# SunYangtian/Splatter_A_Video

Hardware: AMD Instinct MI355X
Metric: rendered frames/sec fwd+bwd @480p, 300k Gaussians (higher is better)
Workload: dtype f32

## Files before the change

### splatter_a_video_amd/csrc/blend.hip

```cpp
#include <stdlib.h>

#include <utility>

#include "common.h"

__device__ __forceinline__ float exp2_guard(float pw, bool &ok) {
    ok = true;
    return __builtin_amdgcn_fmed3f(__builtin_amdgcn_exp2f(pw), 0.f, 1.f);
}

struct BlendArgs {
    int P, C;
    int c0, cn;
    const float2 *uv;
    const float *conic;
    const float *opacity;
    const float *feature;
    const float *bias;
    const int *idx_sorted;
    const int2 *tile_range;
    float bg;
    const float *bgc;
    int W, H, gx;
    int K, trunc;
// ... 352 lines not shown
__device__ __forceinline__ void keep_from_flags(TileLDS<CH, SB, COEF, XR, SWZ, RQL> &L, int tid, int nb, unsigned flags, Pred pred) {
    if (tid < SB) {
        unsigned kw = 0u;
        if (tid < nb) {
#pragma unroll
            for (int ww = 0; ww < 4; ++ww)
                if (((flags >> (8 * ww)) & 0xffu) && pred(tid, ww)) kw |= 1u << (8 * ww);
        }
        L.keep[tid] = kw;
    }
}

template <int SB, bool POS = true>
struct CarryLDS {
    static constexpr int CQ = 15;
    unsigned int pos4[POS ? SB : 1];
    int cslot[4][16];
    int more[4];
};

template <int CH, int SB, bool COEF, int XR, bool SWZ, int RQL, bool POS>
__device__ __forceinline__ int build_list_at(TileLDS<CH, SB, COEF, XR, SWZ, RQL> &L, CarryLDS<SB, POS> &C, int w, int lane, int base) {
    int cnt = 0;
#pragma unroll
    for (int r = 0; r < SB / WAVE; ++r) {
        const int e = r * WAVE + lane;
        const bool keep = ((L.keep[e] >> (8 * w)) & 0xffu) != 0u;
        const unsigned long long m = __ballot(keep);
        const int before = __builtin_amdgcn_mbcnt_hi((unsigned)(m >> 32), __builtin_amdgcn_mbcnt_lo((unsigned)m, 0u));
        if (keep) L.list[w][base + cnt + before] = (unsigned short)e;
        if (POS) reinterpret_cast<unsigned char *>(C.pos4)[4 * e + w] = keep ? (unsigned char)(base + cnt + before) : (unsigned char)255;
        cnt += __popcll(m);
    }
    if (lane < 16) L.list[w][base + cnt + lane] = (unsigned short)SB;
    __builtin_amdgcn_fence(__ATOMIC_RELEASE, "wavefront");
    __builtin_amdgcn_wave_barrier();
    return cnt;
}

template <int CH, int SB, bool COEF, int XR, bool SWZ, bool POS>
__device__ __forceinline__ void carry_out(TileLDS<CH, SB, COEF, XR, SWZ> &L, CarryLDS<SB, POS> &C, int w, int lane, int first, int left,
                                          int j0, int top, const int *slots) {
    constexpr int RQC = 2 + (CH + 3) / 4, CQ = CarryLDS<SB>::CQ;
    for (int idx = lane; idx < left * RQC; idx += WAVE) {
        const int k = idx / RQC, part = idx - k * RQC;
        const int e = L.list[w][first + k];
        float4 v = L.rec[L.part(e, part)];
        if (part == 1) v.w = __int_as_float(top - e);
        L.rec[L.part(SB + 1 + CQ * w + j0 + k, part)] = v;
    }
    int e = 0;
    if (lane < left) {
        e = L.list[w][first + lane];
        C.cslot[w][j0 + lane] = slots[top - e];
        if (POS) reinterpret_cast<unsigned char *>(C.pos4)[4 * e + w] = (unsigned char)255;
    }
    __builtin_amdgcn_fence(__ATOMIC_RELEASE, "wavefront");
    __builtin_amdgcn_wave_barrier();
    if (lane < left) L.list[w][j0 + lane] = (unsigned short)(SB + 1 + CQ * w + j0 + lane);
}

typedef float f32x4 __attribute__((ext_vector_type(4)));

template <int CH>
struct FwdCfg {
    static constexpr int SB = 128;
    static constexpr int U = 2;
    static constexpr int MINW = CH <= 4 ? 6 : CH <= 16 ? 4 : 3;
};

template <int CH, bool ENH, bool BIAS, bool EXACT>
__global__ void __launch_bounds__(256, FwdCfg<CH>::MINW)
blend_fwd_kernel(const BlendArgs B) {
    constexpr int SB = FwdCfg<CH>::SB;
    constexpr bool MF = CH >= 16 && !BIAS;
    constexpr int NCB = (CH + 15) / 16;
    constexpr int U = MF ? 4 : FwdCfg<CH>::U;
    constexpr int RB = Rec<CH>::RS * 4;
    constexpr int RM = RB / 32;
    constexpr int CS = (!BIAS && CH <= 4) ? 3 : 2;
    constexpr int CSB = 16 * CS;
    static_assert((SB + 1) * CSB <= 65536 && SB % U == 0 && RB % 32 == 0, "offsets must fit the 16-bit list entries");
    static_assert(BIAS ? CSB == 32 : true, "with a bias the list entries address the records (32-byte unit)");
    __shared__ TileLDS<CH, SB, !BIAS, 0, false, Rec<CH>::RQ, CS> L;
    __shared__ __attribute__((aligned(16))) unsigned int s_qlist[4][4][SB];
    __shared__ int s_done[4];
    const int tid = threadIdx.x, lane = tid & 63, w = tid >> 6;
    const int gtile = xcd_tile(blockIdx.x, gridDim.x);
    const int frame = gtile / B.T, tile = gtile - frame * B.T;
    const BlendArgs A = frame_args(B, frame);
    const int tx = tile % A.gx, ty = tile / A.gx;
    const int bx = tx * TILE + (w & 1) * 8, by = ty * TILE + (w >> 1) * 8;
    const int lx = MF ? ((lane >> 4) & 1) * 4 + (lane & 3) : (lane & 7);
    const int ly = MF ? (lane >> 5) * 4 + ((lane >> 2) & 3) : (lane >> 3);
    const int px = bx + lx, py = by + ly;
    const float pxf = (float)px, pyf = (float)py;
    const float x = (float)((w & 1) * 8 + lx) - 7.5f, y = (float)((w >> 1) * 8 + ly) - 7.5f;
    const float xx = x * x, xy = x * y, yy = y * y;
    const int cn = EXACT ? CH : A.cn;
    f32x4 D[MF ? 4 : 1][MF ? NCB : 1];
    if (MF) {
#pragma unroll
        for (int g = 0; g < 4; ++g)
#pragma unroll
            for (int c = 0; c < NCB; ++c) D[g][c] = f32x4{0.f, 0.f, 0.f, 0.f};
    }

    const bool inside = (px < A.W) && (py < A.H);
    float T = inside ? 1.0f : -1.0f, F[CH];
    int last = 0, layer = 0;
#pragma unroll
    for (int k = 0; k < CH; ++k) F[k] = 0.f;
    const int2 range = A.tile_range[tile];
    const int n = range.y - range.x;

    if (tid < Rec<CH>::RQ) L.rec[SB * Rec<CH>::RQ + tid] = make_float4(0.f, 0.f, 0.f, 0.f);
    if (!BIAS && tid < CS) L.coef[CS * SB + tid] = make_float4(tid == 0 ? -__builtin_inff() : 0.f, 0.f, 0.f, 0.f);
    auto pos = [n](int e, int b) { const int q = b * SB + e; return q < n ? q : -1; };
    Stager<CH, SB> st;
    st.load_ids(A, tid, range.x, pos, 0);
    st.load_payload(A, tid);
    st.load_ids(A, tid, range.x, pos, 1);

    for (int base = 0, batch = 0; base < n; base += SB, ++batch) {
        unsigned qd;
        {
            const unsigned long long dm = __ballot(T < 0.f);
            if (MF) {
                qd = ((dm & 0xffffull) == 0xffffull ? 1u : 0u) | (((dm >> 16) & 0xffffull) == 0xffffull ? 2u : 0u) |
                     (((dm >> 32) & 0xffffull) == 0xffffull ? 4u : 0u) | ((dm >> 48) == 0xffffull ? 8u : 0u);
            } else {
                constexpr unsigned long long Q0 = 0x000000000F0F0F0Full, Q1 = 0x00000000F0F0F0F0ull;
                qd = ((dm & Q0) == Q0 ? 1u : 0u) | ((dm & Q1) == Q1 ? 2u : 0u) | ((dm & (Q0 << 32)) == (Q0 << 32) ? 4u : 0u) |
                     ((dm & (Q1 << 32)) == (Q1 << 32) ? 8u : 0u);
            }
        }
        const bool alld = qd == 15u;
        if (lane == 0) s_done[w] = (int)qd;
        const int nb = imin_(SB, n - base);
        st.park(L, tid);
        st.load_payload(A, tid);
        st.load_ids(A, tid, range.x, pos, batch + 2);
        __syncthreads();
        if ((s_done[0] & s_done[1] & s_done[2] & s_done[3]) == 15) break;
        tile_cull<CH, SB, BIAS, true, !BIAS>(L, tid, nb, (float)(tx * TILE), (float)(ty * TILE), [&](int, int ww) -> unsigned { return 15u & ~(unsigned)s_done[ww]; },
                                             A.cull_flags ? A.cull_flags + range.x + base : nullptr);
        __syncthreads();
        if (!alld) {
            int cq[4];
#pragma unroll
            for (int q = 0; q < 4; ++q) cq[q] = 0;
#pragma unroll
            for (int r = 0; r < SB / WAVE; ++r) {
                const int e = r * WAVE + lane;
                const unsigned bits = (L.keep[e] >> (8 * w)) & 0xffu;
#pragma unroll
                for (int q = 0; q < 4; ++q) {
                    const bool keep = (bits >> q) & 1u;
                    const unsigned long long m = __ballot(keep);
                    const int before = __builtin_amdgcn_mbcnt_hi((unsigned)(m >> 32), __builtin_amdgcn_mbcnt_lo((unsigned)m, 0u));
                    if (keep) s_qlist[w][q][cq[q] + before] = (unsigned)(e * CSB);
                    cq[q] += __popcll(m);
                }
            }
            const int cnt = imax_(imax_(cq[0], cq[1]), imax_(cq[2], cq[3]));
            const int cntU = (cnt + U - 1) / U * U;
#pragma unroll
            for (int q = 0; q < 4; ++q)
#pragma unroll 1
                for (int i = cq[q] + lane; i < cntU; i += WAVE) s_qlist[w][q][i] = (unsigned)(SB * CSB);
            __builtin_amdgcn_fence(__ATOMIC_RELEASE, "wavefront");
            __builtin_amdgcn_wave_barrier();
            const int myq = MF ? (lane >> 4) : ((lane >> 2) & 1) + 2 * ((lane >> 5) & 1);
            const unsigned int *mylist = s_qlist[w][myq];
            const char *recb = reinterpret_cast<const char *>(L.rec);
            const char *cfb = reinterpret_cast<const char *>(L.coef);
            int lastoff = -1;
            const int chan_off = 4 * (lane & 15);
            const int chan_off1 = (16 + (lane & 15) < CH) ? 64 : -chan_off;
            for (int j0 = 0; j0 < cntU; j0 += U) {
                unsigned off[U];
                static_assert(U == 2 || U == 4, "a trip reads its list entries as one 8- or 16-byte word");
#pragma unroll
                for (int u = 0; u < U; ++u) off[u] = mylist[j0 + u];
                float bq[MF ? 4 : 1][MF ? NCB : 1];
                if constexpr (MF) {
#pragma unroll
                    for (int g = 0; g < 4; ++g) {
                        const unsigned og = s_qlist[w][g][j0 + (lane >> 4)];
                        const char *fb = recb + og * RM + 32 + chan_off;
#pragma unroll
                        for (int c = 0; c < NCB; ++c) bq[g][c] = *reinterpret_cast<const float *>(fb + (c == 0 ? 0 : chan_off1));
                    }
                }
                float4 g0[U], g1[U];
                float alpha[U];
                bool aok[U];
#pragma unroll
                for (int u = 0; u < U; ++u) {
                    const char *src = BIAS ? recb + off[u] * RM : cfb + off[u];
                    g0[u] = *reinterpret_cast<const float4 *>(src);
                    g1[u] = *reinterpret_cast<const float4 *>(src + 16);
                }
#pragma unroll
                for (int u = 0; u < U; ++u) {
                    if (BIAS) {
                        const float q = neg_power_factored(g0[u].x - pxf, g0[u].y - pyf, g0[u].z, g0[u].w, g1[u].x);
                        const float a = fminf(0.99f, __builtin_fmaf(g1[u].y, exp_neg(q), g1[u].z));
                        aok[u] = !(q < 0.f) && !(a < (1.0f / 255.0f));
                        alpha[u] = aok[u] ? a : 0.f;
                    } else {
                        const float pw = power_poly(g0[u], g1[u], x, y, xx, xy, yy);
                        bool pw_ok;
                        const float a = fminf(0.99f, exp2_guard(pw, pw_ok));
                        aok[u] = pw_ok && !(a < (1.0f / 255.0f));
                        alpha[u] = aok[u] ? a : 0.f;
                    }
                }
                float wq[MF ? U : 1];
#pragma unroll
                for (int u = 0; u < U; ++u) {
                    float f[MF ? 1 : CH];
                    if (!MF) {
                        if (CS == 3) asm volatile("" : "+v"(off[u]) : "v"(alpha[u]));
                        const float4 *fq = CS == 3 ? reinterpret_cast<const float4 *>(cfb + off[u] + 32)
                                                   : reinterpret_cast<const float4 *>(recb + off[u] * RM + 32);
#pragma unroll
                        for (int k = 0; k < CH; k += 4) {
                            const float4 v = fq[k / 4];
                            if (k + 0 < CH) f[k + 0] = v.x;
                            if (k + 1 < CH) f[k + 1] = v.y;
                            if (k + 2 < CH) f[k + 2] = v.z;
                            if (k + 3 < CH) f[k + 3] = v.w;
                        }
                    }
                    const float nT = T * (1.f - alpha[u]);
                    const bool sat = nT < 0.0001f;
                    const float wgt = sat ? 0.f : alpha[u] * T;
                    const bool app = CH <= 8 ? (aok[u] && !sat) : wgt > 0.f;
                    if (MF) {
                        wq[u] = wgt;
                    } else {
#pragma unroll
                        for (int k = 0; k < CH; ++k) F[k] += f[k] * wgt;
                    }
                    T = sat ? -fabsf(T) : nT;
                    lastoff = app ? (int)off[u] : lastoff;
                    if (ENH) {
                        if (app && (A.trunc || layer < A.K)) {
                            const size_t pix = (size_t)A.W * (size_t)py + px;
                            A.gs_idx[pix * A.K + layer] = __float_as_int(g1[u].w);
                            layer++;
                            if (A.trunc && layer >= A.K) T = -T;
                        }
                    }
                }
                if constexpr (MF) {
                    typedef unsigned u32x2_f __attribute__((ext_vector_type(2)));
                    const u32x2_f s02 = __builtin_amdgcn_permlane32_swap(__float_as_uint(wq[0]), __float_as_uint(wq[2]), false, false);
                    const u32x2_f s13 = __builtin_amdgcn_permlane32_swap(__float_as_uint(wq[1]), __float_as_uint(wq[3]), false, false);
                    const u32x2_f a01 = __builtin_amdgcn_permlane16_swap(s02[0], s13[0], false, false);
                    const u32x2_f a23 = __builtin_amdgcn_permlane16_swap(s02[1], s13[1], false, false);
                    const float Aq[4] = {__uint_as_float(a01[0]), __uint_as_float(a01[1]), __uint_as_float(a23[0]), __uint_as_float(a23[1])};
#pragma unroll
                    for (int g = 0; g < 4; ++g)
#pragma unroll
                        for (int c = 0; c < NCB; ++c) D[g][c] = __builtin_amdgcn_mfma_f32_16x16x4f32(Aq[g], bq[g][c], D[g][c], 0, 0, 0);
                }
            }
            last = lastoff >= 0 ? base + lastoff / CSB + 1 : last;
        }
        __syncthreads();
    }
    if constexpr (MF) {
        constexpr int ST = 36;
        static_assert(4 * 16 * ST * 4 <= (int)sizeof(L.rec), "four waves' quarter buffers fit the staged records");
        float *so = reinterpret_cast<float *>(L.rec) + w * (16 * ST);
#pragma unroll
        for (int g = 0; g < 4; ++g) {
#pragma unroll
            for (int c = 0; c < NCB; ++c)
#pragma unroll
                for (int j = 0; j < 4; ++j) so[(4 * (lane >> 4) + j) * ST + 16 * c + (lane & 15)] = D[g][c][j];
            __builtin_amdgcn_fence(__ATOMIC_RELEASE, "wavefront");
            __builtin_amdgcn_wave_barrier();
            const float4 *src = reinterpret_cast<const float4 *>(so + (lane & 15) * ST);
            const bool mine = (lane >> 4) == g;
#pragma unroll
            for (int k = 0; k < CH; k += 4) {
                const float4 v = src[k / 4];
                if (k + 0 < CH) F[k + 0] = mine ? v.x : F[k + 0];
                if (k + 1 < CH) F[k + 1] = mine ? v.y : F[k + 1];
                if (k + 2 < CH) F[k + 2] = mine ? v.z : F[k + 2];
                if (k + 3 < CH) F[k + 3] = mine ? v.w : F[k + 3];
            }
            __builtin_amdgcn_fence(__ATOMIC_RELEASE, "wavefront");
            __builtin_amdgcn_wave_barrier();
        }
    }
    if (inside) {
        const size_t HW = (size_t)A.H * A.W;
        const size_t pix = (size_t)A.W * (size_t)py + px;
        T = fabsf(T);
        A.final_T[pix] = T;
        A.ncontrib[pix] = last;
#pragma unroll
        for (int k = 0; k < CH; ++k)
            if (k < cn) A.out[(size_t)(A.c0 + k) * HW + pix] = F[k] + T * (A.bgc ? A.bgc[A.c0 + k] : A.bg);
        if (ENH)
            for (int l = layer; l < A.K; ++l) A.gs_idx[pix * A.K + l] = -1;
    }
}

#define DPP4(op)                                   \
    "v_add_f32_dpp %0, %0, %0 " op "\n\t"          \
    "v_add_f32_dpp %1, %1, %1 " op "\n\t"          \
    "v_add_f32_dpp %2, %2, %2 " op "\n\t"          \
    "v_add_f32_dpp %3, %3, %3 " op "\n\t"

__device__ __forceinline__ void wave_sum4_to_lane63(float &a, float &b, float &c, float &d) {
    asm volatile("s_nop 1\n\t" DPP4("row_shr:1 row_mask:0xf bank_mask:0xf bound_ctrl:1")
                     DPP4("row_shr:2 row_mask:0xf bank_mask:0xf bound_ctrl:1")
                         DPP4("row_shr:4 row_mask:0xf bank_mask:0xf bound_ctrl:1")
                             DPP4("row_shr:8 row_mask:0xf bank_mask:0xf bound_ctrl:1")
                                 DPP4("row_bcast:15 row_mask:0xa bank_mask:0xf")
                                     DPP4("row_bcast:31 row_mask:0xc bank_mask:0xf")
                 : "+v"(a), "+v"(b), "+v"(c), "+v"(d));
}

#define DPP3(op)                                   \
    "v_add_f32_dpp %0, %0, %0 " op "\n\t"          \
    "v_add_f32_dpp %1, %1, %1 " op "\n\t"          \
    "v_add_f32_dpp %2, %2, %2 " op "\n\t"

__device__ __forceinline__ void wave_sum3_to_lane63(float &a, float &b, float &c) {
    asm volatile("s_nop 1\n\t" DPP3("row_shr:1 row_mask:0xf bank_mask:0xf bound_ctrl:1")
                     DPP3("row_shr:2 row_mask:0xf bank_mask:0xf bound_ctrl:1")
                         DPP3("row_shr:4 row_mask:0xf bank_mask:0xf bound_ctrl:1")
                             DPP3("row_shr:8 row_mask:0xf bank_mask:0xf bound_ctrl:1")
                                 DPP3("row_bcast:15 row_mask:0xa bank_mask:0xf")
                                     DPP3("row_bcast:31 row_mask:0xc bank_mask:0xf")
                 : "+v"(a), "+v"(b), "+v"(c));
}

template <int N>
__device__ __forceinline__ void wave_sum_n_to_lane63(float (&v)[N]) {
    constexpr int B3 = (N >= 6 || N == 3) ? ((4 - (N & 3)) & 3) : 0;
    constexpr int N3 = 3 * B3;
    constexpr int N4 = (N - N3) & ~3;
#pragma unroll
    for (int k = 0; k < N4; k += 4) wave_sum4_to_lane63(v[k], v[k + 1], v[k + 2], v[k + 3]);
#pragma unroll
    for (int k = N4; k < N4 + N3; k += 3) wave_sum3_to_lane63(v[k], v[k + 1], v[k + 2]);
// ... 674 lines not shown
                        for (int i = 0; i < 4; ++i) {
                            const int c = 16 * q + 4 * kk + i;
                            if (c < CH) put(rec + NG + c, d_f[q][i]);
                        }
                }
            }
        }
        if (CARRY && p0 == 0) {
            __builtin_amdgcn_fence(__ATOMIC_RELEASE, "wavefront");
            __builtin_amdgcn_wave_barrier();
            if (nproc > 0)
                for (int idx = lane; idx < ncin * NC; idx += 64) {
                    const int k = idx / NC, c = idx - k * NC;
                    float *src = SHARED ? slab + (SB + CQ * w + k) * NCS + c : slab + idx;
                    __hip_atomic_fetch_add(pair_buf + (size_t)CL.cslot[w][k] * RST + c, *src, __ATOMIC_RELAXED,
                                           __HIP_MEMORY_SCOPE_AGENT);
                    if (SHARED) *src = 0.f;
                }
            const int left = total - nproc;
            if (left > 0) carry_out<CH, SB>(L, CL, w, lane, nproc > 0 ? nproc : ncin, nproc > 0 ? left : left - ncin,
                                            nproc > 0 ? 0 : ncin, top, slots);
            ncarry = left;
        }
        if (CARRY && !SHARED && lane == 0) CL.more[w] = nproc > p0 + CAP;
        if (p0 == 0) {
            load_slots();
            st.load_payload(A, tid);
            st.load_ids(A, tid, range.x, pos, batch + 2);
        }
        __syncthreads();
        if (ce < EPI) {
            const int lo = top - nb + 1;
            if (SHARED) {
#pragma unroll
                for (int r = 0; r < NPASS; ++r) {
                    const int ql = ce + r * EPI;
                    if (ql < nb) {
                        float *row = s_acc[0] + (nb - 1 - ql) * NCS + CW * cc;
                        const float v0 = row[0], v1 = row[CW > 1 ? 1 : 0], v2 = row[CW > 1 ? 2 : 0];
                        row[0] = 0.f;
                        if (CW > 1) { row[1] = 0.f; row[2] = 0.f; }
                        store_part(NPASS <= 3 ? sl[NPASS <= 3 ? r : 0] : slots[lo + ql], v0, v1, v2);
                    }
                }
            } else {
#pragma unroll
                for (int r = 0; r < NPASS; ++r) {
                    const int ql = ce + r * EPI;
                    if (ql < nb) {
                        const unsigned int p4 = CL.pos4[nb - 1 - ql];
                        float v[3] = {0.f, 0.f, 0.f};
#pragma unroll
                        for (int ww = 0; ww < 4; ++ww) {
                            const unsigned int pp = umin_(((p4 >> (8 * ww)) & 0xffu) - (unsigned)p0, (unsigned)CAP);
                            const float *row = s_acc[ww] + pp * NC + CW * cc;
#pragma unroll
                            for (int j = 0; j < 3; ++j)
                                if (CW * (TPR - 1) + j < NC || CW * cc + j < NC) v[j] += row[j];
                        }
                        const int slot = NPASS <= 3 ? sl[NPASS <= 3 ? r : 0] : slots[lo + ql];
                        if (p0 > 0) {
                            const float *old = pair_buf + (size_t)slot * RST + CW * cc;
#pragma unroll
                            for (int j = 0; j < 3; ++j)
                                if (CW * cc + j < NCP) v[j] += old[j];
                        }
                        store_part(slot, v[0], v[1], v[2]);
                    }
                }
            }
        }
        if (SHARED) break;
        const bool more = CARRY && (CL.more[0] | CL.more[1] | CL.more[2] | CL.more[3]);
        __syncthreads();
        if (!more) break;
        }
    }
    if (A.dbg_T_front) {
        const int px = bx + (lane & 7), py = by + (lane >> 3);
        if (px < A.W && py < A.H) A.dbg_T_front[(size_t)A.W * py + px] = s_pix[w][pixoff(lane) + PS + 2];
    }
}

template <int CH, bool ABS = false>
struct QuarterCfg {
    static_assert(CH <= 3 && Rec<CH>::RQ == 4 && Rec<CH>::CULL >= 11, "floats 11-15 of the record (cull parameters) are free for the coefficients");
    static constexpr int SB = 128;
    static constexpr int CAP = 80;
    static constexpr int MINW = 4;
    static constexpr int NG = GradLayout<ABS, false>::NG, NC = NG + CH, NCP = PAIR_STRIDE(NC);
    static constexpr int RW = ABS ? 16 : 12;
    static constexpr int PW = 8;
};

template <int CH, bool ABS, bool EXACT>
__global__ void __launch_bounds__(256, (QuarterCfg<CH, ABS>::MINW))
blend_bwd_quarter_kernel(const BlendArgs B) {
    using Cfg = QuarterCfg<CH, ABS>;
    constexpr int SB = Cfg::SB, CAP = Cfg::CAP, NCP = Cfg::NCP, RW = Cfg::RW, PW = Cfg::PW, RQ = 4;
    static_assert(SB <= 128 && CAP < 255, "list entries are (entry | position << 8) in 16 bits");
    __shared__ float4 s_rec[(SB + 1) * RQ];
    auto qpart = [](int e, int p) { return 4 * e + (p ^ ((e >> 2) & 3)); };
    __shared__ unsigned int s_keep[SB];
    __shared__ unsigned short s_qlist[4][4][CAP + 16];
    __shared__ unsigned int s_pos4[SB];
    __shared__ __attribute__((aligned(16))) float s_acc[4][(CAP + 1) * RW];
    constexpr int KS = 4 * PW + 8, GS = 4 * KS;
    __shared__ __attribute__((aligned(16))) float s_pix[4][4 * GS];
    auto pixoff = [](int q) { return (q >> 4) * GS + ((q >> 2) & 3) * KS + (q & 3) * PW; };
    __shared__ float s_mom[16 * 32];
    __shared__ int s_wmax[4];
    __shared__ int s_more[4];
    const int tid = threadIdx.x, lane = tid & 63, w = tid >> 6;
    const int gtile = xcd_tile(blockIdx.x, gridDim.x);
    const int frame = gtile / B.T, tile = gtile - frame * B.T;
    const BlendArgs A = frame_args(B, frame);
    const int RST = B.rec_stride ? B.rec_stride : NCP;
    float *const pair_buf = B.pair_buf + (size_t)frame * (size_t)B.cap * RST + B.rec_off;
    const int tx = tile % A.gx, ty = tile / A.gx;
    const int bx = tx * TILE + (w & 1) * 8, by = ty * TILE + (w >> 1) * 8;
    const float tcx = (float)(tx * TILE) + 7.5f, tcy = (float)(ty * TILE) + 7.5f;
    const float ox = (float)((w & 1) * 8) - 7.5f, oy = (float)((w >> 1) * 8) - 7.5f;
    const int cn = EXACT ? CH : A.cn;
    const int nl = lane & 15, kk = lane >> 4;
    auto qx = [](int q) { return 4 * ((q >> 4) & 1) + (q & 3); };
    auto qy = [](int q) { return 4 * (q >> 5) + ((q >> 2) & 3); };
#pragma unroll
    for (int r = 0; r < 4; ++r) {
        const int st = 4 * w + r, Gs = st >> 2, is = st & 3;
        const int q = 16 * Gs + 4 * kk + is;
        const float x = (float)qx(q) - 3.5f, y = (float)qy(q) - 3.5f;
        float v = 0.f;
        if (ABS) {
            if (nl < 4) v = nl == 0 ? 1.f : nl == 1 ? x : nl == 2 ? y : x * x;
            else if (nl < 6) v = nl == 4 ? x * y : y * y;
        } else {
            if (nl < 3) v = nl == 0 ? 1.f : nl == 1 ? x : y;
            else if (nl >= 4 && nl < 7) v = nl == 4 ? x * x : nl == 5 ? x * y : y * y;
        }
        if (nl < 8) s_mom[32 * st + 8 * kk + nl] = v;
    }
    float phi1[4], phi2[4];
#pragma unroll
    for (int Gs = 0; Gs < 4; ++Gs) {
        const int q = 16 * Gs + nl;
        const float x = (float)qx(q) + ox, y = (float)qy(q) + oy;
        phi1[Gs] = kk == 0 ? 1.f : kk == 1 ? x : kk == 2 ? y : x * x;
        phi2[Gs] = kk == 0 ? x * y : kk == 1 ? y * y : 0.f;
    }
    const int lx = lane & 7, ly = lane >> 3;
    const int myq = 16 * ((lx >> 2) + 2 * (ly >> 2)) + 4 * (ly & 3) + (lx & 3);
    {
        const int px = bx + lx, py = by + ly;
        const size_t HW = (size_t)A.H * A.W;
        const bool inside = (px < A.W) && (py < A.H);
        const size_t pix = (size_t)A.W * (size_t)py + px;
        const float Tf = inside ? A.final_T[pix] : 0.f;
        const int last = inside ? A.ncontrib[pix] : 0;
        float *r = s_pix[w] + pixoff(myq);
        float bgdot = 0.f;
#pragma unroll
        for (int k = 0; k < 4; ++k) {
            const float g = (k < CH && inside && k < cn) ? A.dL_dout[(size_t)(A.c0 + k) * HW + pix] : 0.f;
            r[k] = g;
            bgdot += A.bg * g;
        }
        r[4] = 0.f;
        r[5] = __int_as_float(last);
        r[6] = Tf;
        r[7] = Tf * bgdot;
        const int wmax = wave_max_i(last);
        if (lane == 0) s_wmax[w] = wmax;
    }
    if (tid < RQ) s_rec[qpart(SB, tid)] = make_float4(tid == 3 ? -__builtin_inff() : 0.f, 0.f, 0.f, 0.f);
    if (lane < RW) s_acc[w][CAP * RW + lane] = 0.f;
    __syncthreads();
    const int2 range = A.tile_range[tile];
    const int len = range.y - range.x;
    const int n = imin_(len, imax_(imax_(s_wmax[0], s_wmax[1]), imax_(s_wmax[2], s_wmax[3])));
    const int *slots = A.slot_sorted + range.x;
    auto store_rec = [&](int slot, const float (&v)[12]) {
        float4 *dst = reinterpret_cast<float4 *>(pair_buf + (size_t)slot * RST);
#pragma unroll
        for (int c = 0; c < NCP / 4; ++c) dst[c] = make_float4(v[4 * c], v[4 * c + 1], v[4 * c + 2], v[4 * c + 3]);
    };
    {
        const float z[12] = {0.f, 0.f, 0.f, 0.f, 0.f, 0.f, 0.f, 0.f, 0.f, 0.f, 0.f, 0.f};
        for (int ql = n + tid; ql < len; ql += 256) store_rec(slots[ql], z);
    }
    if (n <= 0) {
        if (A.dbg_T_front) {
            const int px = bx + lx, py = by + ly;
            if (px < A.W && py < A.H) A.dbg_T_front[(size_t)A.W * py + px] = s_pix[w][pixoff(myq) + 6];
        }
        return;
    }
    float *pixrow = s_pix[w] + kk * KS;
    const float *pixcol = s_pix[w] + pixoff(nl);
    const float *momrow = s_mom + 8 * kk + (nl & 7);
    const int kch = kk < CH ? kk : 4;

    auto pos = [n](int e, int b) { return n - 1 - b * SB - e; };
    Stager<CH, SB> st;
    static_assert(Stager<CH, SB>::NCHUNK % 256 == 0, "every thread parks K chunks");
    st.load_ids(A, tid, range.x, pos, 0);
    st.load_payload(A, tid);
    st.load_ids(A, tid, range.x, pos, 1);
    auto load_flags = [&](int topb) -> unsigned {
        const int q = topb - tid;
        return (tid < SB && q >= 0) ? (unsigned)A.cull_flags[range.x + q] : 0u;
    };
    unsigned fl_next = load_flags(n - 1);

    int batch = 0;
    for (int top = n - 1; top >= 0; top -= SB, ++batch) {
        const int nb = imin_(SB, top + 1);
        {
            const int p = tid & 3;
#pragma unroll
            for (int k = 0; k < Stager<CH, SB>::K; ++k) {
                const int e = (tid >> 2) + 64 * k;
                const float4 mine = st.v[k];
                float4 other;
                other.x = __int_as_float(__builtin_amdgcn_mov_dpp(__float_as_int(mine.x), 0xB1, 0xf, 0xf, true));
                other.y = __int_as_float(__builtin_amdgcn_mov_dpp(__float_as_int(mine.y), 0xB1, 0xf, 0xf, true));
                other.z = __int_as_float(__builtin_amdgcn_mov_dpp(__float_as_int(mine.z), 0xB1, 0xf, 0xf, true));
                other.w = __int_as_float(__builtin_amdgcn_mov_dpp(__float_as_int(mine.w), 0xB1, 0xf, 0xf, true));
                const float4 g0 = p == 0 ? mine : other, g1 = p == 0 ? other : mine;
                const PowerCoef pc = power_coeffs(g0.x, g0.y, g0.z, g0.w, g1.x, g1.y, tcx, tcy);
                if (p == 0) {
                    s_rec[qpart(e, 0)] = mine;
                    s_rec[qpart(e, 3)] = make_float4(pc.q0, pc.qx, pc.qy, pc.qxx);
                } else if (p == 1) {
                    s_rec[qpart(e, 1)] = make_float4(mine.x, mine.y, pc.qxy, pc.qyy);
                } else if (p == 2) {
                    s_rec[qpart(e, 2)] = make_float4(mine.x, mine.y, mine.z, 0.f);
                }
            }
        }
        const unsigned fl = fl_next;
        fl_next = load_flags(top - SB);
        if (tid < SB) {
            unsigned kw = 0u;
            if (tid < nb) {
#pragma unroll
                for (int ww = 0; ww < 4; ++ww)
                    if (top - tid < s_wmax[ww]) kw |= fl & (0xfu << (8 * ww));
            }
            s_keep[tid] = kw;
        }
        __syncthreads();
        float *slab = s_acc[w];
        int slot_mine = 0;
        for (int p0 = 0;; p0 += CAP) {
            unsigned cqw = 0u;
            int cnt = 0;
#pragma unroll
            for (int r = 0; r < SB / WAVE; ++r) {
                const int e = r * WAVE + lane;
                unsigned bits = (s_keep[e] >> (8 * w)) & 0xfu;
                const bool kb = bits != 0u;
                const unsigned long long m = __builtin_amdgcn_ballot_w64(kb);
                const int ps = cnt + __builtin_amdgcn_mbcnt_hi((unsigned)(m >> 32), __builtin_amdgcn_mbcnt_lo((unsigned)m, 0u));
                if (p0 == 0) reinterpret_cast<unsigned char *>(s_pos4)[4 * e + w] = kb ? (unsigned char)imin_(ps, 254) : (unsigned char)255;
                bits = ((unsigned)(ps - p0) < (unsigned)CAP) ? bits : 0u;
                const unsigned word = (bits * 0x00204081u) & 0x01010101u;
                unsigned incl = word;
                asm volatile("s_nop 1\n\t"
                             "v_add_u32_dpp %0, %0, %0 row_shr:1 row_mask:0xf bank_mask:0xf\n\t"
                             "s_nop 1\n\t"
                             "v_add_u32_dpp %0, %0, %0 row_shr:2 row_mask:0xf bank_mask:0xf\n\t"
                             "s_nop 1\n\t"
                             "v_add_u32_dpp %0, %0, %0 row_shr:4 row_mask:0xf bank_mask:0xf\n\t"
                             "s_nop 1\n\t"
                             "v_add_u32_dpp %0, %0, %0 row_shr:8 row_mask:0xf bank_mask:0xf\n\t"
                             "s_nop 1\n\t"
                             "v_add_u32_dpp %0, %0, %0 row_bcast:15 row_mask:0xa bank_mask:0xf\n\t"
                             "s_nop 1\n\t"
                             "v_add_u32_dpp %0, %0, %0 row_bcast:31 row_mask:0xc bank_mask:0xf\n\t"
                             : "+v"(incl));
                const unsigned posw = cqw + incl - word;
                const unsigned short ent = (unsigned short)(e | ((ps - p0) << 8));
#pragma unroll
                for (int q = 0; q < 4; ++q)
                    if ((bits >> q) & 1u) s_qlist[w][q][(posw >> (8 * q)) & 0xffu] = ent;
                cqw += (unsigned)__builtin_amdgcn_readlane((int)incl, 63);
                cnt += __popcll(m);
            }
            int cq[4];
#pragma unroll
            for (int q = 0; q < 4; ++q) cq[q] = (int)((cqw >> (8 * q)) & 0xffu);
            if (lane < 16) {
#pragma unroll
                for (int q = 0; q < 4; ++q) s_qlist[w][q][cq[q] + lane] = (unsigned short)(SB | (CAP << 8));
            }
            {
                const int rows = imin_(imax_(cnt - p0, 0), CAP);
                float4 *z = reinterpret_cast<float4 *>(slab);
                for (int c = lane; c < rows * (RW / 4); c += WAVE) z[c] = make_float4(0.f, 0.f, 0.f, 0.f);
            }
            if (lane == 0) s_more[w] = cnt > p0 + CAP;
            __builtin_amdgcn_fence(__ATOMIC_RELEASE, "wavefront");
            __builtin_amdgcn_wave_barrier();
#pragma unroll
            for (int G = 0; G < 4; ++G) {
                for (int j0 = 0; j0 < cq[G]; j0 += 16) {
                    const unsigned le = s_qlist[w][G][j0 + nl];
                    const int e = le & 0xffu, row = le >> 8;
                    const int qn = top - e;
                    const float *er = reinterpret_cast<const float *>(s_rec) + e * (4 * RQ);
                    const int sw = 4 * ((e >> 2) & 3);
                    const float bq1 = er[(12 ^ sw) + kk];
                    const float bq2 = er[(4 ^ sw) + 2 + (kk & 1)];
                    const float bf = er[(8 ^ sw) + kk];
                    float blx = 0.f, bly = 0.f;
                    if (ABS) {
                        const float4 ge = *reinterpret_cast<const float4 *>(er + (0 ^ sw));
                        const float cCe = er[(4 ^ sw)];
                        const float ut = ge.x - tcx, vt = ge.y - tcy;
                        blx = kk == 0 ? -(ge.z * ut + ge.w * vt) : kk == 1 ? ge.z : kk == 2 ? ge.w : 0.f;
                        bly = kk == 0 ? -(ge.w * ut + cCe * vt) : kk == 1 ? ge.w : kk == 2 ? cCe : 0.f;
                    }
                    float s_ax = 0.f, s_ay = 0.f;
                    f32x4 d_mom = {0.f, 0.f, 0.f, 0.f};
                    float dfv[CH];
#pragma unroll
                    for (int c = 0; c < CH; ++c) dfv[c] = 0.f;
                    asm volatile("" ::: "memory");
                    f32x4 pw = {0.f, 0.f, 0.f, 0.f}, cgv = {0.f, 0.f, 0.f, 0.f};
                    pw = __builtin_amdgcn_mfma_f32_16x16x4f32(phi1[G], bq1, pw, 0, 0, 0);
                    pw = __builtin_amdgcn_mfma_f32_16x16x4f32(phi2[G], bq2, pw, 0, 0, 0);
                    cgv = __builtin_amdgcn_mfma_f32_16x16x4f32(pixcol[G * GS + kch], bf, cgv, 0, 0, 0);
                    float cg[4], araw[4], a[4], r1a[4], rp[4], Ts4[4], Rs4[4];
                    float4 gq[4];
#pragma unroll
                    for (int i = 0; i < 4; ++i) {
                        gq[i] = *reinterpret_cast<const float4 *>(pixrow + G * GS + i * PW);
                        const float4 stv = *reinterpret_cast<const float4 *>(pixrow + G * GS + i * PW + 4);
                        cg[i] = cgv[i];
                        const int last = __float_as_int(stv.y);
                        Ts4[i] = stv.z;
                        Rs4[i] = stv.w;
                        bool pw_ok;
                        araw[i] = exp2_guard(pw[i], pw_ok);
                        const bool ok = (qn < last) && pw_ok && !(araw[i] < (1.0f / 255.0f));
                        araw[i] = ok ? araw[i] : 0.f;
                        a[i] = fminf(0.99f, araw[i]);
                        r1a[i] = __builtin_amdgcn_rcpf(1.f - a[i]);
                        rp[i] = r1a[i];
                    }
                    row_scan_mul4(rp[0], rp[1], rp[2], rp[3]);
                    float T[4], wgt[4], rs[4], R[4];
#pragma unroll
                    for (int i = 0; i < 4; ++i) {
                        T[i] = Ts4[i] * rp[i];
                        wgt[i] = a[i] * T[i];
                        rs[i] = cg[i] * wgt[i];
                    }
                    row_scan_add4(rs[0], rs[1], rs[2], rs[3]);
                    row_shr1_add4(R, rs, Rs4);
                    lds_store2x4_lane15<6, PW + 6, 2 * PW + 6, 3 * PW + 6>(pixrow + G * GS, T[0], Rs4[0] + rs[0], T[1], Rs4[1] + rs[1], T[2],
                                                                           Rs4[2] + rs[2], T[3], Rs4[3] + rs[3]);
                    f32x4 lx4 = {0.f, 0.f, 0.f, 0.f}, ly4 = {0.f, 0.f, 0.f, 0.f};
                    if (ABS) {
                        lx4 = __builtin_amdgcn_mfma_f32_16x16x4f32(phi1[G], blx, lx4, 0, 0, 0);
                        ly4 = __builtin_amdgcn_mfma_f32_16x16x4f32(phi1[G], bly, ly4, 0, 0, 0);
                    }
#pragma unroll
                    for (int i = 0; i < 4; ++i) {
                        const float dLa = T[i] * cg[i] - R[i] * r1a[i];
                        const float dLp = araw[i] * dLa;
                        d_mom = __builtin_amdgcn_mfma_f32_16x16x4f32(momrow[32 * (4 * G + i)], dLp, d_mom, 0, 0, 0);
                        if (ABS) {
                            s_ax += fabsf(dLp * lx4[i]);
                            s_ay += fabsf(dLp * ly4[i]);
                        }
                        dfv[0] = __builtin_fmaf(gq[i].x, wgt[i], dfv[0]);
                        if (CH > 1) dfv[1 % CH] = __builtin_fmaf(gq[i].y, wgt[i], dfv[1 % CH]);
                        if (CH > 2) dfv[2 % CH] = __builtin_fmaf(gq[i].z, wgt[i], dfv[2 % CH]);
                    }
                    if (ABS) {
                        s_ax = rows_sum(s_ax, lane);
                        s_ay = rows_sum(s_ay, lane);
                    }
                    float fs[3] = {0.f, 0.f, 0.f};
#pragma unroll
                    for (int c = 0; c < CH; ++c) {
                        const u32x2_b r = __builtin_amdgcn_permlane32_swap(__float_as_uint(dfv[c]), __float_as_uint(dfv[c]), false, false);
                        fs[c] = __uint_as_float(r[0]) + __uint_as_float(r[1]);
                    }
                    if (!ABS) {
                        if (j0 + nl < cq[G]) {
                            F3 *r3 = reinterpret_cast<F3 *>(slab + row * RW + 3 * kk);
                            F3 v3 = *r3;
                            v3.x += kk < 2 ? d_mom[0] : fs[0];
                            v3.y += kk < 2 ? d_mom[1] : fs[1];
                            v3.z += kk < 2 ? d_mom[2] : fs[2];
                            *r3 = v3;
                        }
                    } else if (kk < 2 && j0 + nl < cq[G]) {
                        float4 *rm = reinterpret_cast<float4 *>(slab + row * RW + 4 * kk), *rf = rm + 2;
                        float4 m4 = *rm, f4 = *rf;
                        m4.x += d_mom[0]; m4.y += d_mom[1];
                        m4.z += ABS ? d_mom[2] + (kk == 1 ? s_ax : 0.f) : d_mom[2];
                        m4.w += ABS ? d_mom[3] + (kk == 1 ? s_ay : 0.f) : d_mom[3];
                        f4.x += fs[0]; f4.y += fs[1]; f4.z += fs[2];
                        *rm = m4;
                        *rf = f4;
                    }
                    __builtin_amdgcn_fence(__ATOMIC_RELEASE, "wavefront");
                    __builtin_amdgcn_wave_barrier();
                }
            }
            if (p0 == 0) {
                slot_mine = tid < nb ? slots[top - tid] : 0;
                st.load_payload(A, tid);
                st.load_ids(A, tid, range.x, pos, batch + 2);
            }
            __syncthreads();
            if (tid < nb) {
                const int e = tid;
                const unsigned int p4 = s_pos4[e];
                float s[12] = {0.f, 0.f, 0.f, 0.f, 0.f, 0.f, 0.f, 0.f, 0.f, 0.f, 0.f, 0.f};
#pragma unroll
                for (int ww = 0; ww < 4; ++ww) {
                    const unsigned int pp = umin_(((p4 >> (8 * ww)) & 0xffu) - (unsigned)p0, (unsigned)CAP);
                    const float4 *rw = reinterpret_cast<const float4 *>(s_acc[ww] + pp * RW);
                    float4 m, m2, fa, fb;
                    if (ABS) {
                        m = rw[0]; m2 = rw[1]; fa = rw[2]; fb = rw[3];
                    } else {
                        const float4 r1 = rw[1], r2 = rw[2];
                        m = rw[0];
                        m2 = make_float4(r1.x, r1.y, 0.f, 0.f);
                        fa = make_float4(r1.z, r1.w, r2.x, 0.f);
                        fb = make_float4(r2.y, r2.z, r2.w, 0.f);
                    }
                    const float bxw = (ww & 1) ? 4.f : -4.f, byw = (ww >> 1) ? 4.f : -4.f;
                    s[0] += m.x;
                    s[1] += m.y + bxw * m.x;
                    s[2] += m.z + byw * m.x;
                    s[3] += m.w + 2.f * bxw * m.y + (bxw * bxw) * m.x;
                    s[4] += m2.x + bxw * m.z + byw * m.y + (bxw * byw) * m.x;
                    s[5] += m2.y + 2.f * byw * m.z + (byw * byw) * m.x;
                    s[6] += fa.x + fb.x; s[7] += fa.y + fb.y; s[8] += fa.z + fb.z;
                    s[9] += m2.z; s[10] += m2.w;
                }
                const float4 g0 = s_rec[qpart(e, 0)], g1 = s_rec[qpart(e, 1)];
                const float cA = g0.z, cB = g0.w, cC = g1.x, o = g1.y;
                const float uc = g0.x - tcx, vc = g0.y - tcy;
                const float M0 = s[0], Mx = s[1], My = s[2], Mxx = s[3], Mxy = s[4], Myy = s[5];
                float rec[12];
                rec[0] = cA * Mx + cB * My - (cA * uc + cB * vc) * M0;
                rec[1] = cB * Mx + cC * My - (cB * uc + cC * vc) * M0;
                rec[2] = -0.5f * (uc * uc * M0 - 2.f * uc * Mx + Mxx);
                rec[3] = -(uc * vc * M0 - uc * My - vc * Mx + Mxy);
                rec[4] = -0.5f * (vc * vc * M0 - 2.f * vc * My + Myy);
                rec[5] = o > 0.f ? M0 / o : 0.f;
                rec[6] = 0.f; rec[7] = 0.f; rec[8] = 0.f; rec[9] = 0.f; rec[10] = 0.f; rec[11] = 0.f;
                if (ABS) { rec[6] = s[9]; rec[7] = s[10]; }
                rec[Cfg::NG] = s[6];
                if (CH > 1) rec[Cfg::NG + 1 % CH] = s[7];
// ... 2154 lines not shown
```

Measured before the change: 5198.

## Broadcast Gaussian coefficients across 16-lane rows via DPP in forward and backward blend

For the small-channel forward path (no bias, three coefficient slots), each lane of a 16-lane row now loads one Gaussian's coefficients and the row evaluates 16 Gaussians in turn. Operands are broadcast with v_fmac_f32_dpp row_newbcast instead of every lane reading the same LDS record, and pixels are remapped to a quad layout so 4x4 pixel quarters share a row. The backward quarter kernel likewise loads per-pixel gradient and last index once per lane and broadcasts them with DPP, replacing per-iteration float4 LDS reads. This is meant to cut LDS read traffic and bank pressure, at the cost of inline-asm DPP sequences, padding lists to multiples of 16, and a switch-based lane select inside the unrolled loops.

```diff
diff --git a/splatter_a_video_amd/csrc/blend.hip b/splatter_a_video_amd/csrc/blend.hip
--- a/splatter_a_video_amd/csrc/blend.hip
+++ b/splatter_a_video_amd/csrc/blend.hip
@@ -458,6 +458,10 @@
     constexpr int CSB = 16 * CS;
     static_assert((SB + 1) * CSB <= 65536 && SB % U == 0 && RB % 32 == 0, "offsets must fit the 16-bit list entries");
     static_assert(BIAS ? CSB == 32 : true, "with a bias the list entries address the records (32-byte unit)");
+    constexpr bool BC = !MF && CS == 3;
+    constexpr bool QM = MF || BC;
+    constexpr int FW = BC ? 16 : U;
+    static_assert(SB % FW == 0, "a padded list fits its SB entries");
     __shared__ TileLDS<CH, SB, !BIAS, 0, false, Rec<CH>::RQ, CS> L;
     __shared__ __attribute__((aligned(16))) unsigned int s_qlist[4][4][SB];
     __shared__ int s_done[4];
@@ -467,11 +471,11 @@
     const BlendArgs A = frame_args(B, frame);
     const int tx = tile % A.gx, ty = tile / A.gx;
     const int bx = tx * TILE + (w & 1) * 8, by = ty * TILE + (w >> 1) * 8;
-    const int lx = MF ? ((lane >> 4) & 1) * 4 + (lane & 3) : (lane & 7);
-    const int ly = MF ? (lane >> 5) * 4 + ((lane >> 2) & 3) : (lane >> 3);
+    const int lx = QM ? ((lane >> 4) & 1) * 4 + (lane & 3) : (lane & 7);
+    const int ly = QM ? (lane >> 5) * 4 + ((lane >> 2) & 3) : (lane >> 3);
     const int px = bx + lx, py = by + ly;
     const float pxf = (float)px, pyf = (float)py;
-    const float x = (float)((w & 1) * 8 + lx) - 7.5f, y = (float)((w >> 1) * 8 + ly) - 7.5f;
+    float x = (float)((w & 1) * 8 + lx) - 7.5f, y = (float)((w >> 1) * 8 + ly) - 7.5f;
     const float xx = x * x, xy = x * y, yy = y * y;
     const int cn = EXACT ? CH : A.cn;
     f32x4 D[MF ? 4 : 1][MF ? NCB : 1];
@@ -502,7 +506,7 @@
         unsigned qd;
         {
             const unsigned long long dm = __ballot(T < 0.f);
-            if (MF) {
+            if (QM) {
                 qd = ((dm & 0xffffull) == 0xffffull ? 1u : 0u) | (((dm >> 16) & 0xffffull) == 0xffffull ? 2u : 0u) |
                      (((dm >> 32) & 0xffffull) == 0xffffull ? 4u : 0u) | ((dm >> 48) == 0xffffull ? 8u : 0u);
             } else {
@@ -541,110 +545,168 @@
             }
             const int cnt = imax_(imax_(cq[0], cq[1]), imax_(cq[2], cq[3]));
             const int cntU = (cnt + U - 1) / U * U;
+            const int cntF = (cnt + FW - 1) / FW * FW;
 #pragma unroll
             for (int q = 0; q < 4; ++q)
 #pragma unroll 1
-                for (int i = cq[q] + lane; i < cntU; i += WAVE) s_qlist[w][q][i] = (unsigned)(SB * CSB);
+                for (int i = cq[q] + lane; i < cntF; i += WAVE) s_qlist[w][q][i] = (unsigned)(SB * CSB);
             __builtin_amdgcn_fence(__ATOMIC_RELEASE, "wavefront");
             __builtin_amdgcn_wave_barrier();
-            const int myq = MF ? (lane >> 4) : ((lane >> 2) & 1) + 2 * ((lane >> 5) & 1);
+            const int myq = QM ? (lane >> 4) : ((lane >> 2) & 1) + 2 * ((lane >> 5) & 1);
             const unsigned int *mylist = s_qlist[w][myq];
             const char *recb = reinterpret_cast<const char *>(L.rec);
             const char *cfb = reinterpret_cast<const char *>(L.coef);
-            int lastoff = -1;
-            const int chan_off = 4 * (lane & 15);
-            const int chan_off1 = (16 + (lane & 15) < CH) ? 64 : -chan_off;
-            for (int j0 = 0; j0 < cntU; j0 += U) {
-                unsigned off[U];
-                static_assert(U == 2 || U == 4, "a trip reads its list entries as one 8- or 16-byte word");
-#pragma unroll
-                for (int u = 0; u < U; ++u) off[u] = mylist[j0 + u];
-                float bq[MF ? 4 : 1][MF ? NCB : 1];
-                if constexpr (MF) {
-#pragma unroll
-                    for (int g = 0; g < 4; ++g) {
-                        const unsigned og = s_qlist[w][g][j0 + (lane >> 4)];
-                        const char *fb = recb + og * RM + 32 + chan_off;
-#pragma unroll
-                        for (int c = 0; c < NCB; ++c) bq[g][c] = *reinterpret_cast<const float *>(fb + (c == 0 ? 0 : chan_off1));
-                    }
-                }
-                float4 g0[U], g1[U];
-                float alpha[U];
-                bool aok[U];
-#pragma unroll
-                for (int u = 0; u < U; ++u) {
-                    const char *src = BIAS ? recb + off[u] * RM : cfb + off[u];
-                    g0[u] = *reinterpret_cast<const float4 *>(src);
-                    g1[u] = *reinterpret_cast<const float4 *>(src + 16);
-                }
-#pragma unroll
-                for (int u = 0; u < U; ++u) {
-                    if (BIAS) {
-                        const float q = neg_power_factored(g0[u].x - pxf, g0[u].y - pyf, g0[u].z, g0[u].w, g1[u].x);
-                        const float a = fminf(0.99f, __builtin_fmaf(g1[u].y, exp_neg(q), g1[u].z));
-                        aok[u] = !(q < 0.f) && !(a < (1.0f / 255.0f));
-                        alpha[u] = aok[u] ? a : 0.f;
-                    } else {
-                        const float pw = power_poly(g0[u], g1[u], x, y, xx, xy, yy);
+            if constexpr (BC) {
+                int lastrel = -(1 << 20);
+                int j0 = 0;
+                asm volatile("" : "+v"(x), "+v"(y));
+                const float xx = x * x, xy = x * y, yy = y * y;
+                const unsigned int *mine = mylist + (lane & 15);
+                for (; j0 < cntU; j0 += 16, lastrel -= 16) {
+                    const unsigned off = mine[j0];
+                    const float4 c0 = *reinterpret_cast<const float4 *>(cfb + off);
+                    const float4 c1 = *reinterpret_cast<const float4 *>(cfb + off + 16);
+                    const float4 c2 = *reinterpret_cast<const float4 *>(cfb + off + 32);
+                    const float fc[4] = {c2.x, c2.y, c2.z, c2.w};
+                    const int rem = cntU - j0;
+                    auto eval = [&](auto uc) {
+                        constexpr int u = decltype(uc)::value;
+                        float pw;
+                        asm("s_nop 1\n\t"
+                            "v_mov_b32_dpp %0, %1 row_newbcast:%c12 row_mask:0xf bank_mask:0xf\n\t"
+                            "v_fmac_f32_dpp %0, %2, %7 row_newbcast:%c12 row_mask:0xf bank_mask:0xf\n\t"
+                            "v_fmac_f32_dpp %0, %3, %8 row_newbcast:%c12 row_mask:0xf bank_mask:0xf\n\t"
+                            "v_fmac_f32_dpp %0, %4, %9 row_newbcast:%c12 row_mask:0xf bank_mask:0xf\n\t"
+                            "v_fmac_f32_dpp %0, %5, %10 row_newbcast:%c12 row_mask:0xf bank_mask:0xf\n\t"
+                            "v_fmac_f32_dpp %0, %6, %11 row_newbcast:%c12 row_mask:0xf bank_mask:0xf"
+                            : "=&v"(pw)
+                            : "v"(c0.x), "v"(c0.y), "v"(c0.z), "v"(c0.w), "v"(c1.x), "v"(c1.y), "v"(x), "v"(y), "v"(xx), "v"(xy), "v"(yy), "n"(u));
                         bool pw_ok;
                         const float a = fminf(0.99f, exp2_guard(pw, pw_ok));
-                        aok[u] = pw_ok && !(a < (1.0f / 255.0f));
-                        alpha[u] = aok[u] ? a : 0.f;
-                    }
-                }
-                float wq[MF ? U : 1];
-#pragma unroll
-                for (int u = 0; u < U; ++u) {
-                    float f[MF ? 1 : CH];
-                    if (!MF) {
-                        if (CS == 3) asm volatile("" : "+v"(off[u]) : "v"(alpha[u]));
-                        const float4 *fq = CS == 3 ? reinterpret_cast<const float4 *>(cfb + off[u] + 32)
-                                                   : reinterpret_cast<const float4 *>(recb + off[u] * RM + 32);
-#pragma unroll
-                        for (int k = 0; k < CH; k += 4) {
-                            const float4 v = fq[k / 4];
-                            if (k + 0 < CH) f[k + 0] = v.x;
-                            if (k + 1 < CH) f[k + 1] = v.y;
-                            if (k + 2 < CH) f[k + 2] = v.z;
-                            if (k + 3 < CH) f[k + 3] = v.w;
+                        const bool aok = pw_ok && !(a < (1.0f / 255.0f));
+                        const float alpha = aok ? a : 0.f;
+                        const float nT = T * (1.f - alpha);
+                        const bool sat = nT < 0.0001f;
+                        const float wgt = sat ? 0.f : alpha * T;
+                        const bool app = aok && !sat;
+#pragma unroll
+                        for (int k = 0; k < CH; ++k)
+                            asm("v_fmac_f32_dpp %0, %1, %2 row_newbcast:%c3 row_mask:0xf bank_mask:0xf" : "+v"(F[k]) : "v"(fc[k]), "v"(wgt), "n"(u));
+                        T = sat ? -fabsf(T) : nT;
+                        lastrel = app ? u : lastrel;
+                        if (ENH) {
+                            const int id = __builtin_amdgcn_update_dpp(0, __float_as_int(c1.w), 0x150 + u, 0xf, 0xf, true);
+                            if (app && (A.trunc || layer < A.K)) {
+                                const size_t pix = (size_t)A.W * (size_t)py + px;
+                                A.gs_idx[pix * A.K + layer] = id;
+                                layer++;
+                                if (A.trunc && layer >= A.K) T = -T;
+                            }
+                        }
+                    };
+#define FWD_EVAL2(u) eval(std::integral_constant<int, u>{}); eval(std::integral_constant<int, u + 1>{});
+#define FWD_NEXT2(u) if (rem <= u) break; FWD_EVAL2(u)
+                    FWD_EVAL2(0) FWD_NEXT2(2) FWD_NEXT2(4) FWD_NEXT2(6) FWD_NEXT2(8) FWD_NEXT2(10) FWD_NEXT2(12) FWD_NEXT2(14)
+#undef FWD_NEXT2
+#undef FWD_EVAL2
+                }
+                const int lastpos = j0 + lastrel;
+                const int lastoff = (int)mine[imax_(lastpos, 0) - (lane & 15)];
+                last = lastpos >= 0 ? base + lastoff / CSB + 1 : last;
+            } else {
+                int lastoff = -1;
+                const int chan_off = 4 * (lane & 15);
+                const int chan_off1 = (16 + (lane & 15) < CH) ? 64 : -chan_off;
+                for (int j0 = 0; j0 < cntU; j0 += U) {
+                    unsigned off[U];
+                    static_assert(U == 2 || U == 4, "a trip reads its list entries as one 8- or 16-byte word");
+#pragma unroll
+                    for (int u = 0; u < U; ++u) off[u] = mylist[j0 + u];
+                    float bq[MF ? 4 : 1][MF ? NCB : 1];
+                    if constexpr (MF) {
+#pragma unroll
+                        for (int g = 0; g < 4; ++g) {
+                            const unsigned og = s_qlist[w][g][j0 + (lane >> 4)];
+                            const char *fb = recb + og * RM + 32 + chan_off;
+#pragma unroll
+                            for (int c = 0; c < NCB; ++c) bq[g][c] = *reinterpret_cast<const float *>(fb + (c == 0 ? 0 : chan_off1));
                         }
                     }
-                    const float nT = T * (1.f - alpha[u]);
-                    const bool sat = nT < 0.0001f;
-                    const float wgt = sat ? 0.f : alpha[u] * T;
-                    const bool app = CH <= 8 ? (aok[u] && !sat) : wgt > 0.f;
-                    if (MF) {
-                        wq[u] = wgt;
-                    } else {
-#pragma unroll
-                        for (int k = 0; k < CH; ++k) F[k] += f[k] * wgt;
+                    float4 g0[U], g1[U];
+                    float alpha[U];
+                    bool aok[U];
+#pragma unroll
+                    for (int u = 0; u < U; ++u) {
+                        const char *src = BIAS ? recb + off[u] * RM : cfb + off[u];
+                        g0[u] = *reinterpret_cast<const float4 *>(src);
+                        g1[u] = *reinterpret_cast<const float4 *>(src + 16);
                     }
-                    T = sat ? -fabsf(T) : nT;
-                    lastoff = app ? (int)off[u] : lastoff;
-                    if (ENH) {
-                        if (app && (A.trunc || layer < A.K)) {
-                            const size_t pix = (size_t)A.W * (size_t)py + px;
-                            A.gs_idx[pix * A.K + layer] = __float_as_int(g1[u].w);
-                            layer++;
-                            if (A.trunc && layer >= A.K) T = -T;
+#pragma unroll
+                    for (int u = 0; u < U; ++u) {
+                        if (BIAS) {
+                            const float q = neg_power_factored(g0[u].x - pxf, g0[u].y - pyf, g0[u].z, g0[u].w, g1[u].x);
+                            const float a = fminf(0.99f, __builtin_fmaf(g1[u].y, exp_neg(q), g1[u].z));
+                            aok[u] = !(q < 0.f) && !(a < (1.0f / 255.0f));
+                            alpha[u] = aok[u] ? a : 0.f;
+                        } else {
+                            const float pw = power_poly(g0[u], g1[u], x, y, xx, xy, yy);
+                            bool pw_ok;
+                            const float a = fminf(0.99f, exp2_guard(pw, pw_ok));
+                            aok[u] = pw_ok && !(a < (1.0f / 255.0f));
+                            alpha[u] = aok[u] ? a : 0.f;
                         }
                     }
-                }
-                if constexpr (MF) {
-                    typedef unsigned u32x2_f __attribute__((ext_vector_type(2)));
-                    const u32x2_f s02 = __builtin_amdgcn_permlane32_swap(__float_as_uint(wq[0]), __float_as_uint(wq[2]), false, false);
-                    const u32x2_f s13 = __builtin_amdgcn_permlane32_swap(__float_as_uint(wq[1]), __float_as_uint(wq[3]), false, false);
-                    const u32x2_f a01 = __builtin_amdgcn_permlane16_swap(s02[0], s13[0], false, false);
-                    const u32x2_f a23 = __builtin_amdgcn_permlane16_swap(s02[1], s13[1], false, false);
-                    const float Aq[4] = {__uint_as_float(a01[0]), __uint_as_float(a01[1]), __uint_as_float(a23[0]), __uint_as_float(a23[1])};
-#pragma unroll
-                    for (int g = 0; g < 4; ++g)
-#pragma unroll
-                        for (int c = 0; c < NCB; ++c) D[g][c] = __builtin_amdgcn_mfma_f32_16x16x4f32(Aq[g], bq[g][c], D[g][c], 0, 0, 0);
-                }
-            }
-            last = lastoff >= 0 ? base + lastoff / CSB + 1 : last;
+                    float wq[MF ? U : 1];
+#pragma unroll
+                    for (int u = 0; u < U; ++u) {
+                        float f[MF ? 1 : CH];
+                        if (!MF) {
+                            const float4 *fq = reinterpret_cast<const float4 *>(recb + off[u] * RM + 32);
+#pragma unroll
+                            for (int k = 0; k < CH; k += 4) {
+                                const float4 v = fq[k / 4];
+                                if (k + 0 < CH) f[k + 0] = v.x;
+                                if (k + 1 < CH) f[k + 1] = v.y;
+                                if (k + 2 < CH) f[k + 2] = v.z;
+                                if (k + 3 < CH) f[k + 3] = v.w;
+                            }
+                        }
+                        const float nT = T * (1.f - alpha[u]);
+                        const bool sat = nT < 0.0001f;
+                        const float wgt = sat ? 0.f : alpha[u] * T;
+                        const bool app = CH <= 8 ? (aok[u] && !sat) : wgt > 0.f;
+                        if (MF) {
+                            wq[u] = wgt;
+                        } else {
+#pragma unroll
+                            for (int k = 0; k < CH; ++k) F[k] += f[k] * wgt;
+                        }
+                        T = sat ? -fabsf(T) : nT;
+                        lastoff = app ? (int)off[u] : lastoff;
+                        if (ENH) {
+                            if (app && (A.trunc || layer < A.K)) {
+                                const size_t pix = (size_t)A.W * (size_t)py + px;
+                                A.gs_idx[pix * A.K + layer] = __float_as_int(g1[u].w);
+                                layer++;
+                                if (A.trunc && layer >= A.K) T = -T;
+                            }
+                        }
+                    }
+                    if constexpr (MF) {
+                        typedef unsigned u32x2_f __attribute__((ext_vector_type(2)));
+                        const u32x2_f s02 = __builtin_amdgcn_permlane32_swap(__float_as_uint(wq[0]), __float_as_uint(wq[2]), false, false);
+                        const u32x2_f s13 = __builtin_amdgcn_permlane32_swap(__float_as_uint(wq[1]), __float_as_uint(wq[3]), false, false);
+                        const u32x2_f a01 = __builtin_amdgcn_permlane16_swap(s02[0], s13[0], false, false);
+                        const u32x2_f a23 = __builtin_amdgcn_permlane16_swap(s02[1], s13[1], false, false);
+                        const float Aq[4] = {__uint_as_float(a01[0]), __uint_as_float(a01[1]), __uint_as_float(a23[0]), __uint_as_float(a23[1])};
+#pragma unroll
+                        for (int g = 0; g < 4; ++g)
+#pragma unroll
+                            for (int c = 0; c < NCB; ++c) D[g][c] = __builtin_amdgcn_mfma_f32_16x16x4f32(Aq[g], bq[g][c], D[g][c], 0, 0, 0);
+                    }
+                }
+                last = lastoff >= 0 ? base + lastoff / CSB + 1 : last;
+            }
         }
         __syncthreads();
     }
@@ -1485,6 +1547,24 @@
     }
 }
 
+#define ROW_LANES(X) X(0) X(1) X(2) X(3) X(4) X(5) X(6) X(7) X(8) X(9) X(10) X(11) X(12) X(13) X(14) X(15)
+__device__ __forceinline__ void fmac_row_lane(int n, float &acc, float src, float w) {
+    switch (n) {
+#define ROW_CASE(N) case N: asm("v_fmac_f32_dpp %0, %1, %2 row_newbcast:" #N " row_mask:0xf bank_mask:0xf" : "+v"(acc) : "v"(src), "v"(w)); break;
+        ROW_LANES(ROW_CASE)
+#undef ROW_CASE
+    }
+}
+__device__ __forceinline__ int row_lane(int n, int v) {
+    switch (n) {
+#define ROW_CASE(N) case N: return __builtin_amdgcn_update_dpp(0, v, 0x150 + N, 0xf, 0xf, true);
+        ROW_LANES(ROW_CASE)
+#undef ROW_CASE
+    }
+    return v;
+}
+#undef ROW_LANES
+
 template <int CH, bool ABS = false>
 struct QuarterCfg {
     static_assert(CH <= 3 && Rec<CH>::RQ == 4 && Rec<CH>::CULL >= 11, "floats 11-15 of the record (cull parameters) are free for the coefficients");
@@ -1599,6 +1679,13 @@
         return;
     }
     float *pixrow = s_pix[w] + kk * KS;
+    float gpix[3];
+    int lastpix;
+    {
+        const float *r = s_pix[w] + (nl >> 2) * GS + kk * KS + (nl & 3) * PW;
+        gpix[0] = r[0]; gpix[1] = r[1]; gpix[2] = r[2];
+        lastpix = __float_as_int(r[5]);
+    }
     const float *pixcol = s_pix[w] + pixoff(nl);
     const float *momrow = s_mom + 8 * kk + (nl & 7);
     const int kch = kk < CH ? kk : 4;
@@ -1735,15 +1822,13 @@
                     pw = __builtin_amdgcn_mfma_f32_16x16x4f32(phi2[G], bq2, pw, 0, 0, 0);
                     cgv = __builtin_amdgcn_mfma_f32_16x16x4f32(pixcol[G * GS + kch], bf, cgv, 0, 0, 0);
                     float cg[4], araw[4], a[4], r1a[4], rp[4], Ts4[4], Rs4[4];
-                    float4 gq[4];
 #pragma unroll
                     for (int i = 0; i < 4; ++i) {
-                        gq[i] = *reinterpret_cast<const float4 *>(pixrow + G * GS + i * PW);
-                        const float4 stv = *reinterpret_cast<const float4 *>(pixrow + G * GS + i * PW + 4);
+                        const float2 stv = *reinterpret_cast<const float2 *>(pixrow + G * GS + i * PW + 6);
                         cg[i] = cgv[i];
-                        const int last = __float_as_int(stv.y);
-                        Ts4[i] = stv.z;
-                        Rs4[i] = stv.w;
+                        const int last = row_lane(4 * G + i, lastpix);
+                        Ts4[i] = stv.x;
+                        Rs4[i] = stv.y;
                         bool pw_ok;
                         araw[i] = exp2_guard(pw[i], pw_ok);
                         const bool ok = (qn < last) && pw_ok && !(araw[i] < (1.0f / 255.0f));
@@ -1778,9 +1863,9 @@
                             s_ax += fabsf(dLp * lx4[i]);
                             s_ay += fabsf(dLp * ly4[i]);
                         }
-                        dfv[0] = __builtin_fmaf(gq[i].x, wgt[i], dfv[0]);
-                        if (CH > 1) dfv[1 % CH] = __builtin_fmaf(gq[i].y, wgt[i], dfv[1 % CH]);
-                        if (CH > 2) dfv[2 % CH] = __builtin_fmaf(gq[i].z, wgt[i], dfv[2 % CH]);
+#pragma unroll
+                        for (int c = 0; c < CH; ++c)
+                            fmac_row_lane(4 * G + i, dfv[c], gpix[c], wgt[i]);
                     }
                     if (ABS) {
                         s_ax = rows_sum(s_ax, lane);
```

New measurement: 5294 (median of 6 runs). +1.8%, better.
